# Derek-TH-Wang/OpenRoboRL

Hardware: AMD Instinct MI355X
Metric: env steps/sec at N parallel robots (higher is better)
Workload: dtype f32

## Files before the change

### openroborl_amd/csrc/orr_env_kernels.h

```cpp
#pragma once
#if defined(ORR_PHASE_TIMERS) && !defined(ORR_WAVE_TIMELINE)
#define ORR_WAVE_TIMELINE 1
#endif
#ifndef ORR_TU_MAIN
#undef ORR_PHASE_TIMERS
#endif
#include <hip/hip_runtime.h>
#include <type_traits>
#include <math.h>
#include <stdint.h>
#include <stdio.h>
#include <stdlib.h>
#include <string.h>

#include "orr_device.h"

#ifdef ORR_PHASE_TIMERS
__device__ long long g_phase_cycles[orr::kPhaseSlots];
__device__ long long g_wave_phases[2048 * 40];
#define PT_INIT() do { if (threadIdx.x == 0) { for (int i_ = 0; i_ < orr::kPhaseSlots; i_++) S.pt_acc[i_] = 0; S.pt_last = clock64(); } } while (0)
#define PT(k) do { if (threadIdx.x == 0) { const long long t_ = clock64(); S.pt_acc[k] += t_ - S.pt_last; S.pt_last = clock64(); } } while (0)
#define PT_FLUSH() do { if (threadIdx.x == 0 && blockIdx.x == gridDim.x / 2) for (int i_ = 0; i_ < orr::kPhaseSlots; i_++) atomicAdd((unsigned long long*)&g_phase_cycles[i_], (unsigned long long)S.pt_acc[i_]); \
                        if (threadIdx.x == 0 && blockIdx.x < 2048) for (int i_ = 0; i_ < orr::kPhaseSlots; i_++) g_wave_phases[blockIdx.x * 40 + i_] = S.pt_acc[i_]; } while (0)
#else
// ... 168 lines not shown
    const bool any_bad = ((__ballot(bad_act) >> (sub * kLanes)) & ((1ull << (kLanes - 1)) * 2ull - 1ull)) != 0ull;
    if (lane == 0 && any_bad) S.s[kHead - 1] = 1.0f;
  }
  if (lane < 12) {
    const float act = act_in + m_init;
    S.s[O(LAST_ACTION) + lane] = act;
    float x1 = S.s[O(XHIST) + lane], x2 = S.s[O(XHIST) + 12 + lane], y1 = S.s[O(YHIST) + lane], y2 = S.s[O(YHIST) + 12 + lane];
    if (geti(S, O(STATE_ACTION_COUNTER)) == 0) {
      const float d = map_pi(S.co[lane]);
      x1 = x2 = y1 = y2 = d;
    }
    const float y = act * P.fb[0] + (x1 * P.fb[1] + x2 * P.fb[2]) - (y1 * P.fa[1] + y2 * P.fa[2]);
    S.s[O(XHIST) + 12 + lane] = x1; S.s[O(XHIST) + lane] = act;
    S.s[O(YHIST) + 12 + lane] = y1; S.s[O(YHIST) + lane] = y;
    S.s[O(ACTION) + lane] = y;
  }
  WSYNC();
  PT(1);
  int fall = 0;
  const float inv_repeat = 1.0f / (float)c.action_repeat;
  const RingLatency rlat = ring_latency(P, S);
  const float m_gain = m_tsign * S.s[O(STRENGTH) + ml];
  const float m_target = S.s[O(ACTION) + ml], m_prev = S.s[O(FILTER_ACTION) + ml];
  const bool m_has_prev = geti(S, O(FILTER_VALID)) != 0;
  int action_counter = geti(S, O(STATE_ACTION_COUNTER));
  RingCursor ring = {geti(S, O(RING_HEAD)), geti(S, O(RING_LEN))};
  OwnCoord X;
  load_own_coord(S, lane, X);
  int limit_idle = 0;
  const int prio_phase = WPE == 2 ? (int)(((unsigned)wave_id / (unsigned)(P.simds > 0 ? P.simds : 1)) & 1u) : 0;
  const bool prio_turns = WPE == 2 && ((((unsigned)gridDim.x + (unsigned)(P.simds > 0 ? P.simds : 1) - 1u) /
                                        (unsigned)(P.simds > 0 ? P.simds : 1)) & 1u) == 0u;
  float co_own = S.co[ml], qm_c = (S.s[O(Q) + mj] - m_off) * m_dir, qdm_c = S.s[O(QD) + mj] * m_dir;
  for (int sstep = 0; sstep < c.action_repeat; sstep++) {
    constexpr int kPrioTurn = 4, kPrioHi = 1, kPrioOffset = 1, kPrioEqualFrom = 1000;
    if (WPE == 2 && prio_turns) { if (sstep < kPrioEqualFrom && ((((sstep + kPrioOffset) / kPrioTurn) ^ prio_phase) & 1)) __builtin_amdgcn_s_setprio(kPrioHi); else __builtin_amdgcn_s_setprio(0); }
    {
      const float lerp = (float)(sstep + 1) * inv_repeat;
      const float cur = map_pi(co_own);
      const float prev = m_has_prev ? m_prev : cur;
      float cmd = prev + lerp * (m_target - prev);
      cmd = fminf(fmaxf(cmd, cur - c.max_angle_change), cur + c.max_angle_change);
      S.tau[lane < 12 ? mj : lane] = m_gain * (-1.0f * (m_kp * (qm_c - cmd)) - m_kd * qdm_c);
    }
    WSYNC();
    action_counter++;
    PT(2);
    {
      RingFetch F;
      ring_prefetch(rlat, rec, ring, lane, F);
      if constexpr ((MODE & 3) == 2) {
        const size_t slot = (size_t)robot * c.action_repeat + sstep;
        if (lane < 12 && valid) RP.tau_out[slot * 12 + lane] = S.tau[mj] * m_tsign;
        WSYNC();
        for (int i = lane; i < 37; i += kLanes) S.s[O(POS) + i] = RP.traj[slot * 37 + i];
        WSYNC();
        fall = RP.fall[robot];
      } else
      fall = physics_substep<ANCHOR>(P, S, K, lane, sub, sstep == c.action_repeat - 1, X, limit_idle, ANCHOR ? &AS : nullptr, anchor_robot);
      accumulate_contacts();
      qm_c = (S.s[O(Q) + mj] - m_off) * m_dir;
      qdm_c = S.s[O(QD) + mj] * m_dir;
      ring_push_and_ctrl_obs(rec, S, lane, valid, F, ring, qm_c, &co_own);
    }
    PT(10);
  }
  if (WPE == 2) __builtin_amdgcn_s_setprio(3);
  const ResetConst RC = load_reset_const(P, S, lane);
  if (lane == 0) {
    seti(S, O(RING_HEAD), ring.head); seti(S, O(RING_LEN), ring.len);
    seti(S, O(STATE_ACTION_COUNTER), action_counter);
    seti(S, O(FILTER_VALID), 1);
    seti(S, O(STEP_COUNTER), geti(S, O(STEP_COUNTER)) + 1);
  }
  if (lane < 12) S.s[O(FILTER_ACTION) + lane] = m_target;
  WSYNC();
  sensors_push(S, lane, false);
  PT(11);
  const DevClip& clip = S.clip;
  double t = motion_time(P, S);
  double t_phase = t;
  bool switched = false;
  if constexpr (CLIPS) {
    if (t >= (double)clip_change) {
      typedef const int __attribute__((address_space(1)))* gip;
      typedef const float __attribute__((address_space(1)))* gfp;
      const int type = geti(S, O(ROBOT_TYPE));
      const int set_n = ((gip)&P.tab->clip_set_n[0])[type];
      const float sw_min = ((gfp)&P.tab->clip_switch[type][0])[0], sw_max = ((gfp)&P.tab->clip_switch[type][0])[1];
      if (set_n > 1 && sw_max < INFINITY) {
        float u4[4];
        philox_block(c.seed, (uint32_t)geti(S, O(ROBOT_INDEX)), (uint32_t)geti(S, O(EPISODE_IDX)), 8u + (uint32_t)geti(S, O(EP_STEP)), u4);
        const uint32_t m = (uint32_t)(u4[0] * 16777216.0f);
        const int k = (int)((m * (uint32_t)set_n) >> 24);
        const int id = ((gip)&P.tab->clip_set[type][0])[k];
        clip_change = clip_change_time(t, sw_min, sw_max, u4[1]);
// ... 363 lines not shown
```

### openroborl_amd/csrc/orr_physics.h

```cpp
#pragma once


__device__ __forceinline__ void chol6(const float A[36], float L[21], float invdiag[6]) {
#pragma unroll
  for (int i = 0; i < 6; i++) {
#pragma unroll
    for (int j = 0; j <= i; j++) {
      float s = A[i * 6 + j];
#pragma unroll
      for (int k = 0; k < j; k++) s -= L[i * (i + 1) / 2 + k] * L[j * (j + 1) / 2 + k];
      if (i == j) {
        const float rs = rsq(s);
        L[i * (i + 1) / 2 + j] = s * rs;
        invdiag[i] = rs;
      } else {
        L[i * (i + 1) / 2 + j] = s * invdiag[j];
      }
    }
  }
}
__device__ __forceinline__ void chol6_solve(const float L[21], const float invdiag[6], const float b[6], float x[6]) {
  float y[6];
#pragma unroll
  for (int i = 0; i < 6; i++) {
// ... 50 lines not shown
  const pk2 c3b = a3b * r3;
  d4a = pk_nfma(c3b, c3b.x, d4a);
  d5 = fmaf(-c3b.y, c3b.y, d5);
  const float r4 = rsq(d4a.x);
  const float l54 = d4a.y * r4;
  d5 = fmaf(-l54, l54, d5);
  F.idg[0] = r0; F.idg[1] = r1; F.idg[2] = r2; F.idg[3] = r3; F.idg[4] = r4; F.idg[5] = rsq(d5);
  F.l10 = l10; F.l32 = l32; F.l54 = l54;
  F.c0a = c0a; F.c0b = c0b; F.c1a = c1a; F.c1b = c1b; F.c2b = c2b; F.c3b = c3b;
}
__device__ __forceinline__ void chol6_solve_pk(const Chol6Pk& F, float b0, float b1, pk2 b23, pk2 b45, float x[6]) {
  float y[6];
  y[0] = b0 * F.idg[0];
  b1 = fmaf(-F.l10, y[0], b1); b23 = pk_nfma(F.c0a, y[0], b23); b45 = pk_nfma(F.c0b, y[0], b45);
  y[1] = b1 * F.idg[1];
  b23 = pk_nfma(F.c1a, y[1], b23); b45 = pk_nfma(F.c1b, y[1], b45);
  y[2] = b23.x * F.idg[2];
  b23.y = fmaf(-F.l32, y[2], b23.y); b45 = pk_nfma(F.c2b, y[2], b45);
  y[3] = b23.y * F.idg[3];
  b45 = pk_nfma(F.c3b, y[3], b45);
  y[4] = b45.x * F.idg[4];
  b45.y = fmaf(-F.l54, y[4], b45.y);
  y[5] = b45.y * F.idg[5];
  x[5] = y[5] * F.idg[5];
  x[4] = fmaf(-F.l54, x[5], y[4]) * F.idg[4];
  x[3] = fmaf(-F.c3b.y, x[5], fmaf(-F.c3b.x, x[4], y[3])) * F.idg[3];
  x[2] = fmaf(-F.c2b.y, x[5], fmaf(-F.c2b.x, x[4], fmaf(-F.l32, x[3], y[2]))) * F.idg[2];
  x[1] = fmaf(-F.c1b.y, x[5], fmaf(-F.c1b.x, x[4], fmaf(-F.c1a.y, x[3], fmaf(-F.c1a.x, x[2], y[1])))) * F.idg[1];
  x[0] = fmaf(-F.c0b.y, x[5], fmaf(-F.c0b.x, x[4], fmaf(-F.c0a.y, x[3], fmaf(-F.c0a.x, x[2], fmaf(-F.l10, x[1], y[0]))))) * F.idg[0];
}

#ifdef ORR_TU_STEP_W2
constexpr bool kCarrySubtreeMass = false, kOwnLegFactor = false, kPackedVelocityUpdate = false;
#define ORR_COMMON(x) (x)
#define ORR_RARE(x) (x)
#else
constexpr bool kCarrySubtreeMass = true, kOwnLegFactor = true, kPackedVelocityUpdate = true;
#define ORR_COMMON(x) __builtin_expect(!!(x), 1)
#define ORR_RARE(x) __builtin_expect(!!(x), 0)
#endif
struct LegConst {
  float r[3][3], jdir[3], joff[3];
  float com[3], m, Ic[6];
  float msub;
  float damp_l, damp_a;
  float jdir_own, joff_own;
  float int_c0, int_c1;
};
struct OwnCoord { float x0, x1; };
__device__ __forceinline__ void load_own_coord(const Shared& S, int lane, OwnCoord& X) {
  X.x0 = lane < 3 ? 0.0f : (lane < 6 ? S.s[O(POS) + lane - 3] : S.s[O(Q) + lane - 6]);
  X.x1 = lane < 2 ? S.s[O(Q) + 10 + lane] : 0.0f;
}
__device__ __forceinline__ float part_suffix_sum(float x);
__device__ static void load_leg_const(const KParams& P, const Shared& S, int lane, LegConst& K) {
  const int leg = lane & 3, part = (lane >> 2) & 3, own = 3 * leg + (part < 3 ? part : 2);
  const ColdPtr mc = model_cold(P, geti(S, O(ROBOT_TYPE)));
#pragma unroll
  for (int k = 0; k < 3; k++) {
    const int j = 3 * leg + k;
    const bool on = k <= part && part < 3;
#pragma unroll
    for (int i = 0; i < 3; i++) K.r[k][i] = on ? S.m.joint_pos[j][i] : 0.0f;
    K.jdir[k] = on ? S.m.jdir[j] : 0.0f;
    K.joff[k] = S.m.joff[j];
  }
  const bool real = part < 3, base = lane == 12;
  const int body = real ? own + 1 : 0;
#pragma unroll
  for (int i = 0; i < 3; i++) K.com[i] = real ? mc->link_com[own][i] : 0.0f;
// ... 86 lines not shown
  float t0, t1, t2;
  if constexpr (WITH_M) {
    asm("v_mov_b32 %0, 0\n\tv_mov_b32 %1, 0\n\tv_mov_b32 %2, 0\n\t"
        ORR_H_ADD("%0", "%4", "4", "0xb") ORR_H_ADD("%1", "%5", "4", "0xb") ORR_H_ADD("%2", "%6", "4", "0xb")
        "v_fmac_f32 %0, %3, %7\n\tv_fmac_f32 %1, %3, %8\n\tv_fmac_f32 %2, %3, %9\n\t"
        ORR_SUBTREE_ADD("%3", "4", "0xb")
        ORR_H_ADD("%0", "%4", "8", "0xd") ORR_H_ADD("%1", "%5", "8", "0xd") ORR_H_ADD("%2", "%6", "8", "0xd")
        ORR_SUBTREE_ADD("%3", "8", "0xd")
        : "=&v"(t0), "=&v"(t1), "=&v"(t2), "+v"(m)
        : "v"(h[0]), "v"(h[1]), "v"(h[2]), "v"(c[0]), "v"(c[1]), "v"(c[2]));
  } else {
    asm("v_mov_b32 %0, 0\n\tv_mov_b32 %1, 0\n\tv_mov_b32 %2, 0\n\t"
        ORR_H_ADD("%0", "%4", "4", "0xb") ORR_H_ADD("%1", "%5", "4", "0xb") ORR_H_ADD("%2", "%6", "4", "0xb")
        "v_fmac_f32 %0, %3, %7\n\tv_fmac_f32 %1, %3, %8\n\tv_fmac_f32 %2, %3, %9\n\t"
        ORR_H_ADD("%0", "%4", "8", "0xd") ORR_H_ADD("%1", "%5", "8", "0xd") ORR_H_ADD("%2", "%6", "8", "0xd")
        : "=&v"(t0), "=&v"(t1), "=&v"(t2)
        : "v"(m), "v"(h[0]), "v"(h[1]), "v"(h[2]), "v"(c[0]), "v"(c[1]), "v"(c[2]));
  }
  h[0] = t0; h[1] = t1; h[2] = t2;
}
#undef ORR_H_ADD
__device__ __forceinline__ void part_suffix_sum_inplace(float (&v)[6]) {
  static_assert(kRPW == 4, "a robot is one DPP row: lane = leg + 4 part, part = DPP bank");
  asm("s_nop 1\n\t"
      ORR_SUBTREE_ADD("%0", "4", "0xb") ORR_SUBTREE_ADD("%1", "4", "0xb") ORR_SUBTREE_ADD("%2", "4", "0xb")
      ORR_SUBTREE_ADD("%3", "4", "0xb") ORR_SUBTREE_ADD("%4", "4", "0xb") ORR_SUBTREE_ADD("%5", "4", "0xb")
      ORR_SUBTREE_ADD("%0", "8", "0xd") ORR_SUBTREE_ADD("%1", "8", "0xd") ORR_SUBTREE_ADD("%2", "8", "0xd")
      ORR_SUBTREE_ADD("%3", "8", "0xd") ORR_SUBTREE_ADD("%4", "8", "0xd") ORR_SUBTREE_ADD("%5", "8", "0xd")
      : "+v"(v[0]), "+v"(v[1]), "+v"(v[2]), "+v"(v[3]), "+v"(v[4]), "+v"(v[5]));
}
#undef ORR_SUBTREE_ADD

struct BaseFactor { Chol6Pk F; };
__device__ static void leg_dynamics(const KParams& P, Shared& S, const LegConst& K, int lane, BaseFactor& BF) {
  const int leg = lane & 3, part = (lane >> 2) & 3;
  float Rb[9];
#pragma unroll
  for (int i = 0; i < 9; i++) Rb[i] = S.Rb[i];
  const float wb[3] = {S.s[O(ANGVEL)], S.s[O(ANGVEL) + 1], S.s[O(ANGVEL) + 2]};
  const float vb[3] = {S.s[O(LINVEL)], S.s[O(LINVEL) + 1], S.s[O(LINVEL) + 2]};
  float Rw[9], d[3] = {0, 0, 0}, Vw[3] = {wb[0], wb[1], wb[2]}, Vv[3] = {vb[0], vb[1], vb[2]};
  float Aa[3] = {0, 0, 0}, Al[3] = {0, 0, 0};
  float s0[3], sv0[3], s1[3], sv1[3], s2[3], sv2[3], ad0, ad1, ad2;
#pragma unroll
  for (int i = 0; i < 9; i++) Rw[i] = Rb[i];
  float sn0, cs0, sn1, cs1, sn2, cs2;
  {
    const int jo = 3 * leg + (part < 3 ? part : 2);
    float sno, cso;
    joint_sincos(K.jdir_own * (S.s[O(Q) + jo] - K.joff_own), &sno, &cso);
    const float sA = __int_as_float(__builtin_amdgcn_update_dpp(0, __float_as_int(sno), 0x114, 0xF, 0xF, true));
    const float cA = __int_as_float(__builtin_amdgcn_update_dpp(0, __float_as_int(cso), 0x114, 0xF, 0xF, true));
    const float sB = __int_as_float(__builtin_amdgcn_update_dpp(0, __float_as_int(sno), 0x118, 0xF, 0xF, true));
    const float cB = __int_as_float(__builtin_amdgcn_update_dpp(0, __float_as_int(cso), 0x118, 0xF, 0xF, true));
    sn0 = __int_as_float(__builtin_amdgcn_update_dpp(__float_as_int(sno), __float_as_int(sno), 0x114, 0xF, 0x2, false));
    sn0 = __int_as_float(__builtin_amdgcn_update_dpp(__float_as_int(sn0), __float_as_int(sno), 0x118, 0xF, 0x4, false));
    cs0 = __int_as_float(__builtin_amdgcn_update_dpp(__float_as_int(cso), __float_as_int(cso), 0x114, 0xF, 0x2, false));
    cs0 = __int_as_float(__builtin_amdgcn_update_dpp(__float_as_int(cs0), __float_as_int(cso), 0x118, 0xF, 0x4, false));
    sn1 = __int_as_float(__builtin_amdgcn_update_dpp(__float_as_int(sno), __float_as_int(sno), 0x114, 0xF, 0x5, true));
    cs1 = __int_as_float(__builtin_amdgcn_update_dpp(__float_as_int(cso), __float_as_int(cso), 0x114, 0xF, 0x4, false));
    cs1 = part == 0 ? 1.0f : cs1;
    (void)sA; (void)cA; (void)sB; (void)cB;
    sn2 = part == 2 ? sno : 0.0f;
    cs2 = part == 2 ? cso : 1.0f;
  }
  float c0k[3];
  joint_down<0>(S, K, 0, 3 * leg, sn0, cs0, Rw, d, Vw, Vv, Aa, Al, s0, sv0, ad0);
  joint_down<1>(S, K, 1, 3 * leg + 1, sn1, cs1, Rw, d, Vw, Vv, Aa, Al, s1, sv1, ad1, c0k);
  joint_down<1, true>(S, K, 2, 3 * leg + 2, sn2, cs2, Rw, d, Vw, Vv, Aa, Al, s2, sv2, ad2, c0k);
  float so[3], svo[3];
#pragma unroll
  for (int i = 0; i < 3; i++) {
    so[i] = part == 0 ? s0[i] : (part == 3 ? 0.0f : s2[i]);
    svo[i] = part == 0 ? sv0[i] : (part == 3 ? 0.0f : sv2[i]);
  }
  const float ado = part == 0 ? ad0 : (part == 1 ? ad1 : ad2);
  {
    LinkCache& L = S.ph.sub.dyn.lc[part < 3 ? 3 * leg + part : 12 + leg];
#pragma unroll
    for (int i = 0; i < 9; i++) L.Rw[i] = Rw[i];
#pragma unroll
    for (int i = 0; i < 3; i++) { L.ow[i] = S.s[O(POS) + i] + d[i]; L.s[i] = so[i]; L.sv[i] = svo[i]; }
  }
  float I[6], h[3], hcom[3], m = K.m, f[6], pacc[6];
  {
    float c[3];
#pragma unroll
    for (int i = 0; i < 3; i++) hcom[i] = c[i] = fmaf(Rw[3 * i], K.com[0], fmaf(Rw[3 * i + 1], K.com[1], fmaf(Rw[3 * i + 2], K.com[2], d[i])));
    h[0] = m * c[0]; h[1] = m * c[1]; h[2] = m * c[2];
    rot_sym_full(Rw, K.Ic, I);
    float Pa[3], Pl[3];
    {
      const float ux = fmaf(Vw[1], c[2], fmaf(-Vw[2], c[1], Vv[0])), uy = fmaf(Vw[2], c[0], fmaf(-Vw[0], c[2], Vv[1]));
      const float uz = fmaf(Vw[0], c[1], fmaf(-Vw[1], c[0], Vv[2]));
      Pl[0] = m * ux; Pl[1] = m * uy; Pl[2] = m * uz;
      const float ax = fmaf(Aa[1], c[2], fmaf(-Aa[2], c[1], Al[0])), ay = fmaf(Aa[2], c[0], fmaf(-Aa[0], c[2], Al[1]));
      const float az = fmaf(Aa[0], c[1], fmaf(-Aa[1], c[0], Al[2]));
      f[3] = fmaf(m, ax, Vw[1] * Pl[2] - Vw[2] * Pl[1]);
      f[4] = fmaf(m, ay, Vw[2] * Pl[0] - Vw[0] * Pl[2]);
      f[5] = fmaf(m, az, Vw[0] * Pl[1] - Vw[1] * Pl[0]);
      symv(I, Vw, Pa);
      float tx = Vw[1] * Pa[2] - Vw[2] * Pa[1], ty = Vw[2] * Pa[0] - Vw[0] * Pa[2], tz = Vw[0] * Pa[1] - Vw[1] * Pa[0];
      tx = fmaf(I[0], Aa[0], fmaf(I[3], Aa[1], fmaf(I[4], Aa[2], tx)));
      ty = fmaf(I[3], Aa[0], fmaf(I[1], Aa[1], fmaf(I[5], Aa[2], ty)));
      tz = fmaf(I[4], Aa[0], fmaf(I[5], Aa[1], fmaf(I[2], Aa[2], tz)));
      f[0] = fmaf(c[1], f[5], fmaf(-c[2], f[4], tx));
      f[1] = fmaf(c[2], f[3], fmaf(-c[0], f[5], ty));
      f[2] = fmaf(c[0], f[4], fmaf(-c[1], f[3], tz));
    }
    const float hc = h[0] * c[0] + h[1] * c[1] + h[2] * c[2];
// ... 16 lines not shown
  part_suffix_sum_first_moment<!kCarrySubtreeMass>(m, hcom, h);
  if (kCarrySubtreeMass) m = K.msub;
  float Fo[6], bo;
  {
    spatial_inertia_mul(I, h, m, so, svo, &Fo[0], &Fo[3]);
    auto dot6 = [](const float a[3], const float b[3], const float x[3], const float y[3]) __attribute__((always_inline)) {
      return fmaf(a[0], x[0], fmaf(a[1], x[1], fmaf(a[2], x[2], fmaf(b[0], y[0], fmaf(b[1], y[1], b[2] * y[2])))));
    };
    bo = S.tau[3 * leg + (part < 3 ? part : 2)] - dot6(so, svo, &f[0], &f[3]);
    const float hc0 = dot6(s0, sv0, &Fo[0], &Fo[3]), hc1 = dot6(s1, sv1, &Fo[0], &Fo[3]), hc2 = dot6(s2, sv2, &Fo[0], &Fo[3]);
    {
      LegExchange& X = S.ph.sub.dyn.legx[leg];
#pragma unroll
      for (int i = 0; i < 6; i++) X.F[part][i] = Fo[i];
      X.b[part] = bo;
      X.Hc[part][0] = hc0; X.Hc[part][1] = hc1; X.Hc[part][2] = hc2;
    }
  }
  WSYNC();
  float b[3];
  pk2 F2[3][3];
  float H00, H01, H02, H11, H12, H22;
  {
    const LegExchange& X = S.ph.sub.dyn.legx[leg];
#pragma unroll
    for (int k = 0; k < 3; k++) {
      static_assert(sizeof(X.F[0]) == 24 && alignof(LegExchange) >= 8, "pairs");
      const pk2* XF = reinterpret_cast<const pk2*>(&X.F[k][0]);
#pragma unroll
      for (int q = 0; q < 3; q++) F2[k][q] = XF[q];
      b[k] = X.b[k];
    }
    H00 = X.Hc[0][0]; H01 = X.Hc[1][0]; H11 = X.Hc[1][1]; H02 = X.Hc[2][0]; H12 = X.Hc[2][1]; H22 = X.Hc[2][2];
  }
  float Hi[6];
  {
    const float c00 = H11 * H22 - H12 * H12, c01 = H02 * H12 - H01 * H22, c02 = H01 * H12 - H02 * H11;
    const float c11 = H00 * H22 - H02 * H02, c12 = H01 * H02 - H00 * H12, c22 = H00 * H11 - H01 * H01;
    const float idet = __builtin_amdgcn_rcpf(H00 * c00 + H01 * c01 + H02 * c02);
    Hi[0] = c00 * idet; Hi[1] = c11 * idet; Hi[2] = c22 * idet; Hi[3] = c01 * idet; Hi[4] = c02 * idet; Hi[5] = c12 * idet;
  }
  const float hq0 = part == 0 ? Hi[0] : (part == 1 ? Hi[3] : (part == 2 ? Hi[4] : 0.0f));
  const float hq1 = part == 0 ? Hi[3] : (part == 1 ? Hi[1] : (part == 2 ? Hi[5] : 0.0f));
  const float hq2 = part == 0 ? Hi[4] : (part == 1 ? Hi[5] : (part == 2 ? Hi[2] : 0.0f));
  float Tq[6];
  pk2 Tq2[3];
#pragma unroll
  for (int q = 0; q < 3; q++) { Tq2[q] = F2[0][q] * hq0 + F2[1][q] * hq1 + F2[2][q] * hq2; Tq[2 * q] = Tq2[q].x; Tq[2 * q + 1] = Tq2[q].y; }
  {
    LegSolve& Q = S.leg[leg];
    float* const tdst = part < 3 ? &Q.T[part][0] : &S.tdump[0];
#pragma unroll
    for (int q = 0; q < 3; q++) reinterpret_cast<pk2*>(tdst)[q] = Tq2[q];
#pragma unroll
    for (int i = 0; i < 6; i++) Q.Hi[i] = Hi[i];
  }
  float a0[6];
  {
    const pk2 Fo23 = {Fo[2], Fo[3]}, Fo45 = {Fo[4], Fo[5]};
    float d0 = fmaf(-Tq[0], Fo[0], Iacc[0]), a10 = fmaf(-Tq[0], Fo[1], Iacc[3]);
    pk2 a0a = pk_nfma(Fo23, Tq[0], pk2{Iacc[4], Hacc[0]}), a0b = pk_nfma(Fo45, Tq[0], pk2{Hacc[1], Hacc[2]});
    float d1 = fmaf(-Tq[1], Fo[1], Iacc[1]);
    pk2 a1a = pk_nfma(Fo23, Tq[1], pk2{Iacc[5], Hacc[3]}), a1b = pk_nfma(Fo45, Tq[1], pk2{Hacc[4], Hacc[5]});
    pk2 d2a = pk_nfma(Fo23, Tq[2], pk2{Iacc[2], Hacc[6]}), a2b = pk_nfma(Fo45, Tq[2], pk2{Hacc[7], Hacc[8]});
    float d3 = fmaf(-Tq[3], Fo[3], Macc[0]);
    pk2 a3b = pk_nfma(Fo45, Tq[3], pk2{Macc[3], Macc[4]});
// ... 142 lines not shown
    else { G.c20 = cr[0]; G.c21 = cr[1]; G.c22 = cr[2]; }
    jl[k] = dir[0] * cr[0] + dir[1] * cr[1] + dir[2] * cr[2];
    rel += jl[k] * S.ustar[6 + 3 * leg + k];
  }
  G.rr0 = rr[0]; G.rr1 = rr[1]; G.rr2 = rr[2];
  const bool active = enable && (knee ? fr > 0.0f : have);
#pragma unroll
  for (int i = 0; i < 6; i++) R.Jb[i] = knee ? 0.0f : Jb[i];
  R.jl[0] = knee ? 0.0f : jl[0]; R.jl[1] = knee ? 0.0f : jl[1]; R.jl[2] = knee ? 1.0f : jl[2];
  const float kpen = normal ? (dist > 0.0f ? inv_dt : (shank ? erp_dt : erp_m)) : 0.0f;
  float rhs = knee ? -uknee : -rel - dist * kpen;
  if constexpr (ANCHOR) rhs -= (d == 1 ? drift_x : (d == 2 ? drift_y : 0.0f)) * (cfg.friction_erp * inv_dt);
  R.rhs = active ? rhs : 0.0f;
  R.cfm = (normal && !shank) ? cfm_m : 0.0f;
  R.nrm_slot = fric ? 16 + leg : -1;
  R.warm = knee ? -1 : 3 * leg + d;
  R.active = active;
  R.jdi = 0.0f; R.lam = 0.0f; R.w = 0.0f; R.lam_n = 0.0f;
  const float hi = knee ? fr * dt : 1e30f, lo = knee ? -fr * dt : 0.0f;
  R.mu_e = (active && fric) ? mu_s * cfg.plane_friction : 0.0f;
  R.hi_c = (active && !fric) ? hi : 0.0f;
  R.lo_c = (active && !fric) ? lo : 0.0f;
}

typedef float v2f __attribute__((ext_vector_type(2)));
__device__ __forceinline__ void row_response(Shared& S, const orr_config& cfg, Row& R, int slot, const BaseFactor& BF) {
  const int leg = R.leg;
  const LegSolve& QL = S.leg[leg];
  float a0[6], mq[12];
  v2f fb2[3], a02[3];
  float prev = S.s[O(LAMBDA) + (R.warm >= 0 ? R.warm : 0)];
  float jl0 = R.jl[0], jl1 = R.jl[1], jl2 = R.jl[2];
  asm("" : "+v"(jl0), "+v"(jl1), "+v"(jl2));
  {
    const v2f* TL = reinterpret_cast<const v2f*>(&QL.T[0][0]);
#pragma unroll
    for (int p = 0; p < 3; p++) {
      float jb0 = R.Jb[2 * p], jb1 = R.Jb[2 * p + 1];
      asm("" : "+v"(jb0), "+v"(jb1));
      const v2f jb = {jb0, jb1};
      fb2[p] = jb - (TL[p] * jl0 + TL[3 + p] * jl1 + TL[6 + p] * jl2);
    }
    chol6_solve_pk(BF.F, fb2[0].x, fb2[0].y, fb2[1], fb2[2], a0);
#pragma unroll
    for (int p = 0; p < 3; p++) a02[p] = v2f{a0[2 * p], a0[2 * p + 1]};
  }
  asm volatile("" : "+v"(prev));
  const float h0 = QL.Hi[0] * jl0 + QL.Hi[3] * jl1 + QL.Hi[4] * jl2;
  const float h1 = QL.Hi[3] * jl0 + QL.Hi[1] * jl1 + QL.Hi[5] * jl2;
  const float h2 = QL.Hi[4] * jl0 + QL.Hi[5] * jl1 + QL.Hi[2] * jl2;
  const v2f dg = fb2[0] * a02[0] + fb2[1] * a02[1] + fb2[2] * a02[2];
  float dgs = dg.x + dg.y;
  asm volatile("" : "+v"(dgs));
  const float own0 = leg == 0 ? 1.0f : 0.0f, own1 = leg == 1 ? 1.0f : 0.0f, own2 = leg == 2 ? 1.0f : 0.0f, own3 = leg == 3 ? 1.0f : 0.0f;
#pragma unroll
  for (int L4 = 0; L4 < 4; L4++) {
    const v2f* TK = reinterpret_cast<const v2f*>(&S.leg[L4].T[0][0]);
    const float own = L4 == 0 ? own0 : (L4 == 1 ? own1 : (L4 == 2 ? own2 : own3));
#pragma unroll
    for (int k = 0; k < 3; k++) {
      const v2f t2 = TK[3 * k] * a02[0] + TK[3 * k + 1] * a02[1] + TK[3 * k + 2] * a02[2];
      const float hk = k == 0 ? h0 : (k == 1 ? h1 : h2);
      mq[3 * L4 + k] = kOwnLegFactor ? fmaf(own, hk, -(t2.x + t2.y)) : ((L4 == leg ? hk : 0.0f) - (t2.x + t2.y));
    }
  }
  const float diag = fmaf(jl0, h0, fmaf(jl1, h1, fmaf(jl2, h2, dgs)));
#pragma unroll
  for (int i = 0; i < 6; i++) S.ph.sub.W[slot][i] = a0[i];
#pragma unroll
  for (int i = 0; i < 12; i++) S.ph.sub.W[slot][6 + i] = mq[i];
#pragma unroll
  for (int i = 0; i < 6; i++) R.wa[i] = a0[i];
#pragma unroll
  for (int i = 0; i < 12; i++) R.wq[i] = mq[i];
  R.jdi = R.active ? __builtin_amdgcn_rcpf(diag + R.cfm) : 0.0f;
  R.rhs *= R.jdi;
  {
    asm volatile("" : "+v"(prev));
    R.lam = (R.active && R.warm >= 0) ? cfg.warmstart_factor * prev : 0.0f;
    R.w = R.cfm * R.lam;
  }
}

template <int I, int N, class F>
__device__ __forceinline__ void static_for(F&& f) {
  if constexpr (I < N) {
    f(std::integral_constant<int, I>{});
    static_for<I + 1, N>(f);
  }
}
template <class F>
__device__ __forceinline__ void for_active_limit_rows(unsigned int mask, F&& f) {
  static_for<0, 4>([&](auto gc) __attribute__((always_inline)) {
    constexpr int g = decltype(gc)::value;
// ... 234 lines not shown
    }
    asm("" : "+v"(AcA[r]), "+v"(AcB[r]));
  };
  static_for<0, 4>([&](auto rc) __attribute__((always_inline)) {
    constexpr int r = decltype(rc)::value;
    finish(rc, A.wq[3 * r + 2], HAS_B ? B.wq[3 * r + 2] : 0.0f);
  });
  if (HAS_B) {
    for_active_limit_rows(mask, [&](auto rc) __attribute__((always_inline)) {
      constexpr int r = decltype(rc)::value;
      const float sg = bcast_lane<r>(B.jl[(r - 4) % 3], sub);
      finish(rc, sg * A.wq[r - 4], sg * B.wq[r - 4]);
    });
  }
  const unsigned int cm = (mask >> 16) & 0xFu;
  static_for<0, 4>([&](auto gc) __attribute__((always_inline)) {
    constexpr int g = decltype(gc)::value;
    if (ORR_COMMON((cm >> g) & 1u)) {
      float ax, ay, az, bx = 0.0f, by = 0.0f, bz = 0.0f;
      dpp_contact_triplet<4 + g>(G.rr0, G.rr1, G.rr2, G.c00, G.c01, G.c02, G.c10, G.c11, G.c12, G.c20, G.c21, G.c22, A.wa[0], A.wa[1], A.wa[2],
                                 A.wa[3], A.wa[4], A.wa[5], A.wq[3 * g], A.wq[3 * g + 1], A.wq[3 * g + 2], ax, ay, az);
      if (HAS_B)
        dpp_contact_triplet<4 + g>(G.rr0, G.rr1, G.rr2, G.c00, G.c01, G.c02, G.c10, G.c11, G.c12, G.c20, G.c21, G.c22, B.wa[0], B.wa[1], B.wa[2],
                                   B.wa[3], B.wa[4], B.wa[5], B.wq[3 * g], B.wq[3 * g + 1], B.wq[3 * g + 2], bx, by, bz);
      finish(std::integral_constant<int, 16 + g>{}, az, bz);
      finish(std::integral_constant<int, 20 + 2 * g>{}, ax, bx);
      finish(std::integral_constant<int, 21 + 2 * g>{}, ay, by);
    }
  });
}

template <bool ANCHOR = false>
__device__ static int physics_substep(const KParams& P, Shared& S, const LegConst& K, int lane, int sub, bool want_fall, OwnCoord& X,
                                      int& limit_idle, AnchorState* AS = nullptr, bool anchor_robot = false) {
  const orr_config& cfg = P.cfg;
  const float dt = cfg.sim_dt, inv_dt = 1.0f / cfg.sim_dt, erp_dt = cfg.contact_erp / cfg.sim_dt;
  int fp_body = 0, fp_n = 0;
  float fp_x = 0.0f, fp_y = 0.0f, fp_z = 0.0f, fp_r = 0.0f;
  if (ORR_RARE(want_fall)) {
    const ColdPtr mc = model_cold(P, geti(S, O(ROBOT_TYPE)));
    static_assert(ORR_MAX_FALL_PROXIES <= kLanes, "one fall proxy per lane");
    fp_body = mc->fall_body[lane]; fp_x = mc->fall_pos[lane][0]; fp_y = mc->fall_pos[lane][1]; fp_z = mc->fall_pos[lane][2]; fp_r = mc->fall_radius[lane];
    fp_n = mc->num_fall;
  }
  BaseFactor BF;
  leg_dynamics(P, S, K, lane, BF);
  WSYNC();
  PT(3);
  asm volatile("" : "+v"(fp_n));
  int fall = 0;
  if (ORR_RARE(want_fall)) {
    bool hit = false;
    if (lane < fp_n) {
      const int b = fp_body;
      const float* Rw = b == 0 ? S.Rb : S.ph.sub.dyn.lc[b - 1].Rw;
      const float oz = b == 0 ? S.s[O(POS) + 2] : S.ph.sub.dyn.lc[b - 1].ow[2];
      const float wz = Rw[6] * fp_x + Rw[7] * fp_y + Rw[8] * fp_z;
      hit = (oz + wz - fp_r) < cfg.contact_margin;
    }
    fall = ((__ballot(hit) >> (sub * kLanes)) & ((1ull << (kLanes - 1)) * 2ull - 1ull)) != 0ull;
  }
  PT(4);

  Row A, B;
  const bool rowlane = lane < 16;
  ContactGeom G;
  row_setup_bank_a<ANCHOR>(S, cfg, rowlane ? (lane < 4 ? lane : lane + 12) : 0, rowlane, dt, inv_dt, erp_dt, A, G, AS, anchor_robot);
  unsigned long long balB = 0ull;
  if (ORR_COMMON(limit_idle > 0)) {
    limit_idle--;
    B.active = false;
  } else {
    float margin = 1e30f;
    row_setup_limit(S, cfg, (rowlane && lane >= 4) ? lane : 4, rowlane && lane >= 4, inv_dt, erp_dt, B, &margin);
    balB = __ballot(B.active);
    const float steps_f = (rowlane && lane >= 4) ? margin * __builtin_amdgcn_rcpf(cfg.max_coord_velocity * dt) - 1.0f : 1e30f;
    int idle = 0;
    if (__ballot(steps_f < 1.0f) == 0ull) idle = 1;
    if (__ballot(steps_f < 2.0f) == 0ull) idle = 2;
// ... 68 lines not shown
      };
      static_for<0, 4>(add_row);
      if (anyB) {
        for_active_limit_rows(mask, add_row);
      }
      static_for<16, 28>(add_row);
    }
    const float vmax = cfg.max_coord_velocity;
    v0 = __builtin_amdgcn_fmed3f(S.ustar[k0] + du0, -vmax, vmax);
    v1 = __builtin_amdgcn_fmed3f(S.ustar[k1] + du1, -vmax, vmax);
  }
  {
    const float w0 = bcast_lane<0>(v0, sub), w1 = bcast_lane<1>(v0, sub), w2 = bcast_lane<2>(v0, sub);
    const float ww = w0 * w0 + w1 * w1 + w2 * w2, h2 = 0.25f * dt * dt * ww;
    const float sc = 0.5f * dt * fmaf(h2, fmaf(h2, fmaf(h2, -1.0f / 5040.0f, 1.0f / 120.0f), -1.0f / 6.0f), 1.0f);
    const float ch = fmaf(h2, fmaf(h2, fmaf(h2, fmaf(h2, 1.0f / 40320.0f, -1.0f / 720.0f), 1.0f / 24.0f), -0.5f), 1.0f);
    const float dq[4] = {w0 * sc, w1 * sc, w2 * sc, ch};
    float qn[4];
    qmul(dq, &S.s[O(QUAT)], qn);
    const float nn = rsq(qn[0] * qn[0] + qn[1] * qn[1] + qn[2] * qn[2] + qn[3] * qn[3]);
    X.x0 = fmaf(dt * v0, K.int_c0, X.x0);
    X.x1 = fmaf(dt * v1, K.int_c1, X.x1);
    float* const dump = &S.ustar[22];
    float* const pv0 = &S.s[lane < 3 ? O(ANGVEL) + lane : (lane < 6 ? O(LINVEL) + lane - 3 : O(QD) + lane - 6)];
    float* const px0 = lane < 3 ? dump : &S.s[lane < 6 ? O(POS) + lane - 3 : O(Q) + lane - 6];
    float* const pv1 = lane < 2 ? &S.s[O(QD) + 10 + lane] : dump;
    float* const px1 = lane < 2 ? &S.s[O(Q) + 10 + lane] : dump;
    float* const pq = lane < 4 ? &S.s[O(QUAT) + lane] : dump;
    WSYNC();
    *pv0 = lane < 6 ? v0 : v0 * K.int_c0;
    *px0 = X.x0;
    *pv1 = v1 * K.int_c1;
    *px1 = X.x1;
    *pq = pick4(lane, qn[0], qn[1], qn[2], qn[3]) * nn;
  }
  WSYNC();
  PT(9);
  return fall;
}
```

### openroborl_amd/csrc/orr_robot_io.h

```cpp
#pragma once

typedef float f4 __attribute__((ext_vector_type(4)));
__device__ static void load_robot(const KParams& P, const float* rec, Shared& S, int lane) {
  {
    static_assert(kHead % 4 == 0 && ORR_STATE_STRIDE % 4 == 0, "16-byte pieces");
    typedef const f4 __attribute__((address_space(1))) * g4ptr;
    const g4ptr src = (g4ptr)reinterpret_cast<const f4*>(rec);
    f4* dst = reinterpret_cast<f4*>(S.s);
    constexpr int kQ = kHead / 4, kIt = (kQ + kLanes - 1) / kLanes;
    f4 tmp[kIt];
#pragma unroll
    for (int k = 0; k < kIt; k++) { const int q = lane + k * kLanes; tmp[k] = src[q < kQ ? q : kQ - 1]; }
#pragma unroll
    for (int k = 0; k < kIt; k++) { const int q = lane + k * kLanes; if (q < kQ) dst[q] = tmp[k]; }
  }
  WSYNC();
  const DevModel& gm = P.tab->model[geti(S, O(ROBOT_TYPE))];
  {
    static_assert(sizeof(DevClip) % 4 == 0 && sizeof(DevClip) / 4 <= kLanes, "one word of the clip header per lane");
    const unsigned int* cg = reinterpret_cast<const unsigned int*>(&P.tab->clip[geti(S, O(CLIP_ID))]);
    unsigned int* cl = reinterpret_cast<unsigned int*>(&S.clip);
    if (lane < (int)(sizeof(DevClip) / 4)) cl[lane] = cg[lane];
  }
  {
// ... 11 lines not shown
  WSYNC();
}

__device__ static void store_robot(float* rec, const Shared& S, int lane, bool valid) {
  if (valid) {
    typedef f4 __attribute__((address_space(1))) * g4ptr;
    const g4ptr dst = (g4ptr)reinterpret_cast<f4*>(rec);
    const f4* src = reinterpret_cast<const f4*>(S.s);
    constexpr int kQ = O(RING) / 4;
#pragma unroll
    for (int k = 0; k < (kQ + kLanes - 1) / kLanes; k++) { const int q = lane + k * kLanes; if (q < kQ) dst[q] = src[q]; }
    if (lane < O(RING) - 4 * kQ) rec[4 * kQ + lane] = S.s[4 * kQ + lane];
  }
}

__device__ static void ctrl_obs(const KParams& P, const float* rec, Shared& S, int lane) {
  const float lat = S.s[O(LATENCY)], dt = P.cfg.sim_dt;
  const int len = geti(S, O(RING_LEN)), head = geti(S, O(RING_HEAD));
  int k0 = 0, k1 = 0;
  float al = 0.0f;
  if (!(lat <= 0.0f || len == 1)) {
    int n = (int)(lat / dt);
    if (n + 1 >= len) { k0 = k1 = len - 1; }
    else { k0 = n; k1 = n + 1; al = (lat - n * dt) / dt; }
  }
  const int i0 = (head - k0 + 2 * ORR_RING_DEPTH) % ORR_RING_DEPTH, i1 = (head - k1 + 2 * ORR_RING_DEPTH) % ORR_RING_DEPTH;
  for (int i = lane; i < 19; i += kLanes) {
    float e0 = rec[O(RING) + i0 * ORR_RING_ENTRY + i], e1 = rec[O(RING) + i1 * ORR_RING_ENTRY + i];
    S.co[i] = (k0 == k1) ? e0 : (1.0f - al) * e0 + al * e1;
  }
  WSYNC();
}

__device__ __forceinline__ void base_rotation(Shared& S, int lane, float rel[4], float Rb[9]) {
  float qi[4];
  qinv(S.m.init_quat, qi);
  qmul(&S.s[O(QUAT)], qi, rel);
  q_to_mat(rel, Rb);
#pragma unroll
  for (int i = 0; i < 9; i++) S.Rb[i] = Rb[i];
}

struct ResetConst {
  int j;
  float off, dir;
  float init;
  float p0;
};
__device__ __forceinline__ ResetConst load_reset_const(const KParams& P, const Shared& S, int lane) {
  const ColdPtr mc = model_cold(P, geti(S, O(ROBOT_TYPE)));
  const int ml = lane < 12 ? lane : 0;
  return ResetConst{mc->joint_of_motor[ml], mc->motor_offset[ml], mc->motor_dir[ml], mc->init_motor_angles[ml], mc->init_pos[lane < 3 ? lane : 0]};
}

__device__ static void receive_obs(const KParams& P, float* rec, Shared& S, int lane, bool valid, const ResetConst& RC, float* entry = nullptr) {
  const int head = (geti(S, O(RING_HEAD)) + 1) % ORR_RING_DEPTH, len = geti(S, O(RING_LEN));
  float rel[4], Rb[9], rate[3];
  base_rotation(S, lane, rel, Rb);
  mtv3(Rb, &S.s[O(ANGVEL)], rate);
  for (int i = lane; i < ORR_RING_ENTRY; i += kLanes) {
    float val = 0.0f;
    if (i < 12) {
      static_assert(kLanes >= 12, "the first pass of the loop covers the twelve motors");
      val = (S.s[O(Q) + RC.j] - RC.off) * RC.dir;
    } else if (i < 16) {
      val = i == 12 ? rel[0] : (i == 13 ? rel[1] : (i == 14 ? rel[2] : rel[3]));
    } else if (i < 19) {
      val = i == 16 ? rate[0] : (i == 17 ? rate[1] : rate[2]);
    }
    if (valid) rec[O(RING) + head * ORR_RING_ENTRY + i] = val;
// ... 16 lines not shown
  int n;
  float al;
  bool none;
};
__device__ __forceinline__ RingLatency ring_latency(const KParams& P, const Shared& S) {
  const float lat = S.s[O(LATENCY)], dt = P.cfg.sim_dt;
  RingLatency L;
  L.none = lat <= 0.0f;
  L.n = (int)(lat / dt);
  L.al = (lat - L.n * dt) / dt;
  return L;
}
struct RingCursor { int head, len; };
__device__ __forceinline__ int ring_wrap_up(int i) { return i >= ORR_RING_DEPTH ? i - ORR_RING_DEPTH : i; }
__device__ __forceinline__ int ring_wrap_down(int i) { return i < 0 ? i + ORR_RING_DEPTH : i; }
__device__ __forceinline__ void ring_prefetch(const RingLatency& L, const float* rec, const RingCursor& C, int lane, RingFetch& F) {
  const int head = ring_wrap_up(C.head + 1);
  const int len = C.len + 1 > ORR_RING_DEPTH ? ORR_RING_DEPTH : C.len + 1;
  int k0 = 0, k1 = 0;
  F.al = 0.0f;
  if (!(L.none || len == 1)) {
    if (L.n + 1 >= len) { k0 = k1 = len - 1; }
    else { k0 = L.n; k1 = L.n + 1; F.al = L.al; }
  }
  F.same = k0 == k1; F.new0 = k0 == 0; F.new1 = k1 == 0;
  const int i0 = ring_wrap_down(head - k0), i1 = ring_wrap_down(head - k1);
  const float* p0 = rec + O(RING) + i0 * ORR_RING_ENTRY;
  const float* p1 = rec + O(RING) + i1 * ORR_RING_ENTRY;
  const int hi = lane < 3 ? 16 + lane : lane;
  F.e0[0] = p0[lane]; F.e0[1] = p0[hi];
  F.e1[0] = p1[lane]; F.e1[1] = p1[hi];
}
__device__ __forceinline__ void ring_push_and_ctrl_obs(float* rec, Shared& S, int lane, bool valid, const RingFetch& F, RingCursor& C,
                                                       float mang, float* co_own = nullptr) {
  static_assert(ORR_RING_ENTRY == 20, "lane mapping below assumes 20-word entries");
  C.head = ring_wrap_up(C.head + 1);
  C.len = C.len + 1 > ORR_RING_DEPTH ? ORR_RING_DEPTH : C.len + 1;
  float rel[4], Rb[9], rate[3];
  base_rotation(S, lane, rel, Rb);
  mtv3(Rb, &S.s[O(ANGVEL)], rate);
  const float va = lane < 12 ? mang : pick4(lane, rel[0], rel[1], rel[2], rel[3]);
  const float vb = pick4(lane, rate[0], rate[1], rate[2], 0.0f);
  const float a0 = F.new0 ? va : F.e0[0], a1 = F.new1 ? va : F.e1[0];
  const float b0 = F.new0 ? vb : F.e0[1], b1 = F.new1 ? vb : F.e1[1];
  const float co_a = F.same ? a0 : (1.0f - F.al) * a0 + F.al * a1;
  S.co[lane] = co_a;
  if (co_own) *co_own = co_a;
  S.co[lane < 3 ? 16 + lane : 19] = F.same ? b0 : (1.0f - F.al) * b0 + F.al * b1;
  WSYNC();
  float* dst = rec + O(RING) + C.head * ORR_RING_ENTRY;
  if (valid) {
    dst[lane] = va;
    dst[lane < 4 ? 16 + lane : lane] = lane < 4 ? vb : va;
  }
}
```

Measured before the change: 21.74 million.

## Carry base state in registers and hoist LDS reads ahead of waits

Keeps the integrated base quaternion and angular velocity in registers and hands them to the observation step, which avoids re-reading them from LDS. The inverse of the initial quaternion is computed once per step instead of once per substep. Rb and the own joint angle are prefetched before the wave sync, the link-cache writes are moved after the Hessian work, and the first leg's T rows are loaded ahead in the contact response so LDS latency overlaps compute. The cost is higher register pressure, and the scheduling barriers could work against the compiler's own ordering.

```diff
diff --git a/openroborl_amd/csrc/orr_env_kernels.h b/openroborl_amd/csrc/orr_env_kernels.h
--- a/openroborl_amd/csrc/orr_env_kernels.h
+++ b/openroborl_amd/csrc/orr_env_kernels.h
@@ -224,7 +224,16 @@
   const bool prio_turns = WPE == 2 && ((((unsigned)gridDim.x + (unsigned)(P.simds > 0 ? P.simds : 1) - 1u) /
                                         (unsigned)(P.simds > 0 ? P.simds : 1)) & 1u) == 0u;
   float co_own = S.co[ml], qm_c = (S.s[O(Q) + mj] - m_off) * m_dir, qdm_c = S.s[O(QD) + mj] * m_dir;
+  BaseHandoff BH;
+  BH.has_qi = kCarryInitQuatInverse;
+  if (BH.has_qi) qinv(S.m.init_quat, BH.qi);
   for (int sstep = 0; sstep < c.action_repeat; sstep++) {
+    LegHead LH;
+    if (kLegHeadAhead) {
+#pragma unroll
+      for (int i = 0; i < 9; i++) LH.Rb[i] = S.Rb[i];
+      LH.q = S.s[O(Q) + 3 * (lane & 3) + (((lane >> 2) & 3) < 3 ? ((lane >> 2) & 3) : 2)];
+    }
     constexpr int kPrioTurn = 4, kPrioHi = 1, kPrioOffset = 1, kPrioEqualFrom = 1000;
     if (WPE == 2 && prio_turns) { if (sstep < kPrioEqualFrom && ((((sstep + kPrioOffset) / kPrioTurn) ^ prio_phase) & 1)) __builtin_amdgcn_s_setprio(kPrioHi); else __builtin_amdgcn_s_setprio(0); }
     {
@@ -236,11 +245,15 @@
       S.tau[lane < 12 ? mj : lane] = m_gain * (-1.0f * (m_kp * (qm_c - cmd)) - m_kd * qdm_c);
     }
     WSYNC();
+    if (kLegHeadAhead)
+      asm volatile("" : "+v"(LH.Rb[0]), "+v"(LH.Rb[1]), "+v"(LH.Rb[2]), "+v"(LH.Rb[3]), "+v"(LH.Rb[4]), "+v"(LH.Rb[5]), "+v"(LH.Rb[6]), "+v"(LH.Rb[7]),
+                        "+v"(LH.Rb[8]), "+v"(LH.q));
     action_counter++;
     PT(2);
     {
       RingFetch F;
       ring_prefetch(rlat, rec, ring, lane, F);
+      constexpr bool kHandoff = kBaseHandoff && (MODE & 3) != 2;
       if constexpr ((MODE & 3) == 2) {
         const size_t slot = (size_t)robot * c.action_repeat + sstep;
         if (lane < 12 && valid) RP.tau_out[slot * 12 + lane] = S.tau[mj] * m_tsign;
@@ -249,11 +262,11 @@
         WSYNC();
         fall = RP.fall[robot];
       } else
-      fall = physics_substep<ANCHOR>(P, S, K, lane, sub, sstep == c.action_repeat - 1, X, limit_idle, ANCHOR ? &AS : nullptr, anchor_robot);
+      fall = physics_substep<ANCHOR>(P, S, K, lane, sub, sstep == c.action_repeat - 1, X, limit_idle, ANCHOR ? &AS : nullptr, anchor_robot, kHandoff ? &BH : nullptr, kLegHeadAhead ? &LH : nullptr);
       accumulate_contacts();
       qm_c = (S.s[O(Q) + mj] - m_off) * m_dir;
       qdm_c = S.s[O(QD) + mj] * m_dir;
-      ring_push_and_ctrl_obs(rec, S, lane, valid, F, ring, qm_c, &co_own);
+      ring_push_and_ctrl_obs(rec, S, lane, valid, F, ring, qm_c, &co_own, kHandoff ? &BH : nullptr);
     }
     PT(10);
   }
diff --git a/openroborl_amd/csrc/orr_physics.h b/openroborl_amd/csrc/orr_physics.h
--- a/openroborl_amd/csrc/orr_physics.h
+++ b/openroborl_amd/csrc/orr_physics.h
@@ -106,10 +106,12 @@
 
 #ifdef ORR_TU_STEP_W2
 constexpr bool kCarrySubtreeMass = false, kOwnLegFactor = false, kPackedVelocityUpdate = false;
+constexpr bool kBaseHandoff = false, kCarryInitQuatInverse = false, kExchangeShadow = false, kLegHeadAhead = false, kRowResponseAhead = false;
 #define ORR_COMMON(x) (x)
 #define ORR_RARE(x) (x)
 #else
 constexpr bool kCarrySubtreeMass = true, kOwnLegFactor = true, kPackedVelocityUpdate = true;
+constexpr bool kBaseHandoff = true, kCarryInitQuatInverse = true, kExchangeShadow = true, kLegHeadAhead = true, kRowResponseAhead = true;
 #define ORR_COMMON(x) __builtin_expect(!!(x), 1)
 #define ORR_RARE(x) __builtin_expect(!!(x), 0)
 #endif
@@ -262,11 +264,11 @@
 #undef ORR_SUBTREE_ADD
 
 struct BaseFactor { Chol6Pk F; };
-__device__ static void leg_dynamics(const KParams& P, Shared& S, const LegConst& K, int lane, BaseFactor& BF) {
+__device__ static void leg_dynamics(const KParams& P, Shared& S, const LegConst& K, int lane, BaseFactor& BF, const LegHead* LH = nullptr) {
   const int leg = lane & 3, part = (lane >> 2) & 3;
   float Rb[9];
 #pragma unroll
-  for (int i = 0; i < 9; i++) Rb[i] = S.Rb[i];
+  for (int i = 0; i < 9; i++) Rb[i] = LH ? LH->Rb[i] : S.Rb[i];
   const float wb[3] = {S.s[O(ANGVEL)], S.s[O(ANGVEL) + 1], S.s[O(ANGVEL) + 2]};
   const float vb[3] = {S.s[O(LINVEL)], S.s[O(LINVEL) + 1], S.s[O(LINVEL) + 2]};
   float Rw[9], d[3] = {0, 0, 0}, Vw[3] = {wb[0], wb[1], wb[2]}, Vv[3] = {vb[0], vb[1], vb[2]};
@@ -278,7 +280,7 @@
   {
     const int jo = 3 * leg + (part < 3 ? part : 2);
     float sno, cso;
-    joint_sincos(K.jdir_own * (S.s[O(Q) + jo] - K.joff_own), &sno, &cso);
+    joint_sincos(K.jdir_own * ((LH ? LH->q : S.s[O(Q) + jo]) - K.joff_own), &sno, &cso);
     const float sA = __int_as_float(__builtin_amdgcn_update_dpp(0, __float_as_int(sno), 0x114, 0xF, 0xF, true));
     const float cA = __int_as_float(__builtin_amdgcn_update_dpp(0, __float_as_int(cso), 0x114, 0xF, 0xF, true));
     const float sB = __int_as_float(__builtin_amdgcn_update_dpp(0, __float_as_int(sno), 0x118, 0xF, 0xF, true));
@@ -305,7 +307,12 @@
     svo[i] = part == 0 ? sv0[i] : (part == 3 ? 0.0f : sv2[i]);
   }
   const float ado = part == 0 ? ad0 : (part == 1 ? ad1 : ad2);
-  {
+  float lc_ow[3];
+  if constexpr (kExchangeShadow) {
+#pragma unroll
+    for (int i = 0; i < 3; i++) lc_ow[i] = S.s[O(POS) + i] + d[i];
+  }
+  if constexpr (!kExchangeShadow) {
     LinkCache& L = S.ph.sub.dyn.lc[part < 3 ? 3 * leg + part : 12 + leg];
 #pragma unroll
     for (int i = 0; i < 9; i++) L.Rw[i] = Rw[i];
@@ -388,6 +395,14 @@
       b[k] = X.b[k];
     }
     H00 = X.Hc[0][0]; H01 = X.Hc[1][0]; H11 = X.Hc[1][1]; H02 = X.Hc[2][0]; H12 = X.Hc[2][1]; H22 = X.Hc[2][2];
+  }
+  if constexpr (kExchangeShadow) {
+    LinkCache& L = S.ph.sub.dyn.lc[part < 3 ? 3 * leg + part : 12 + leg];
+#pragma unroll
+    for (int i = 0; i < 9; i++) L.Rw[i] = Rw[i];
+#pragma unroll
+    for (int i = 0; i < 3; i++) { L.ow[i] = lc_ow[i]; L.s[i] = so[i]; L.sv[i] = svo[i]; }
+    asm volatile("" : "+v"(H00), "+v"(H01), "+v"(H02), "+v"(H11), "+v"(H12), "+v"(H22) : : "memory");
   }
   float Hi[6];
   {
@@ -596,6 +611,12 @@
   float prev = S.s[O(LAMBDA) + (R.warm >= 0 ? R.warm : 0)];
   float jl0 = R.jl[0], jl1 = R.jl[1], jl2 = R.jl[2];
   asm("" : "+v"(jl0), "+v"(jl1), "+v"(jl2));
+  v2f tk0[9];
+  if constexpr (kRowResponseAhead) {
+    const v2f* TK = reinterpret_cast<const v2f*>(&S.leg[0].T[0][0]);
+#pragma unroll
+    for (int i = 0; i < 9; i++) tk0[i] = TK[i];
+  }
   {
     const v2f* TL = reinterpret_cast<const v2f*>(&QL.T[0][0]);
 #pragma unroll
@@ -610,6 +631,7 @@
     for (int p = 0; p < 3; p++) a02[p] = v2f{a0[2 * p], a0[2 * p + 1]};
   }
   asm volatile("" : "+v"(prev));
+  if constexpr (kRowResponseAhead) asm volatile("" : "+v"(tk0[0]), "+v"(tk0[1]), "+v"(tk0[2]), "+v"(tk0[3]), "+v"(tk0[4]), "+v"(tk0[5]), "+v"(tk0[6]), "+v"(tk0[7]), "+v"(tk0[8]));
   const float h0 = QL.Hi[0] * jl0 + QL.Hi[3] * jl1 + QL.Hi[4] * jl2;
   const float h1 = QL.Hi[3] * jl0 + QL.Hi[1] * jl1 + QL.Hi[5] * jl2;
   const float h2 = QL.Hi[4] * jl0 + QL.Hi[5] * jl1 + QL.Hi[2] * jl2;
@@ -623,7 +645,8 @@
     const float own = L4 == 0 ? own0 : (L4 == 1 ? own1 : (L4 == 2 ? own2 : own3));
 #pragma unroll
     for (int k = 0; k < 3; k++) {
-      const v2f t2 = TK[3 * k] * a02[0] + TK[3 * k + 1] * a02[1] + TK[3 * k + 2] * a02[2];
+      const bool pre = kRowResponseAhead && L4 == 0;
+      const v2f t2 = (pre ? tk0[3 * k] : TK[3 * k]) * a02[0] + (pre ? tk0[3 * k + 1] : TK[3 * k + 1]) * a02[1] + (pre ? tk0[3 * k + 2] : TK[3 * k + 2]) * a02[2];
       const float hk = k == 0 ? h0 : (k == 1 ? h1 : h2);
       mq[3 * L4 + k] = kOwnLegFactor ? fmaf(own, hk, -(t2.x + t2.y)) : ((L4 == leg ? hk : 0.0f) - (t2.x + t2.y));
     }
@@ -924,7 +947,7 @@
 
 template <bool ANCHOR = false>
 __device__ static int physics_substep(const KParams& P, Shared& S, const LegConst& K, int lane, int sub, bool want_fall, OwnCoord& X,
-                                      int& limit_idle, AnchorState* AS = nullptr, bool anchor_robot = false) {
+                                      int& limit_idle, AnchorState* AS = nullptr, bool anchor_robot = false, BaseHandoff* BH = nullptr, const LegHead* LH = nullptr) {
   const orr_config& cfg = P.cfg;
   const float dt = cfg.sim_dt, inv_dt = 1.0f / cfg.sim_dt, erp_dt = cfg.contact_erp / cfg.sim_dt;
   int fp_body = 0, fp_n = 0;
@@ -936,7 +959,7 @@
     fp_n = mc->num_fall;
   }
   BaseFactor BF;
-  leg_dynamics(P, S, K, lane, BF);
+  leg_dynamics(P, S, K, lane, BF, LH);
   WSYNC();
   PT(3);
   asm volatile("" : "+v"(fp_n));
@@ -1071,7 +1094,13 @@
     *px0 = X.x0;
     *pv1 = v1 * K.int_c1;
     *px1 = X.x1;
-    *pq = pick4(lane, qn[0], qn[1], qn[2], qn[3]) * nn;
+    if (kBaseHandoff && BH) {
+      BH->q[0] = qn[0] * nn; BH->q[1] = qn[1] * nn; BH->q[2] = qn[2] * nn; BH->q[3] = qn[3] * nn;
+      BH->w[0] = w0; BH->w[1] = w1; BH->w[2] = w2;
+      *pq = pick4(lane, BH->q[0], BH->q[1], BH->q[2], BH->q[3]);
+    } else {
+      *pq = pick4(lane, qn[0], qn[1], qn[2], qn[3]) * nn;
+    }
   }
   WSYNC();
   PT(9);
diff --git a/openroborl_amd/csrc/orr_robot_io.h b/openroborl_amd/csrc/orr_robot_io.h
--- a/openroborl_amd/csrc/orr_robot_io.h
+++ b/openroborl_amd/csrc/orr_robot_io.h
@@ -67,10 +67,14 @@
   WSYNC();
 }
 
-__device__ __forceinline__ void base_rotation(Shared& S, int lane, float rel[4], float Rb[9]) {
+struct BaseHandoff { float q[4], w[3]; float qi[4]; bool has_qi; };
+struct LegHead { float Rb[9], q; };
+__device__ __forceinline__ void base_rotation(Shared& S, int lane, float rel[4], float Rb[9], const BaseHandoff* BH = nullptr) {
   float qi[4];
-  qinv(S.m.init_quat, qi);
-  qmul(&S.s[O(QUAT)], qi, rel);
+  if (BH && BH->has_qi) { qi[0] = BH->qi[0]; qi[1] = BH->qi[1]; qi[2] = BH->qi[2]; qi[3] = BH->qi[3]; }
+  else qinv(S.m.init_quat, qi);
+  if (BH) qmul(BH->q, qi, rel);
+  else qmul(&S.s[O(QUAT)], qi, rel);
   q_to_mat(rel, Rb);
 #pragma unroll
   for (int i = 0; i < 9; i++) S.Rb[i] = Rb[i];
@@ -153,13 +157,13 @@
   F.e1[0] = p1[lane]; F.e1[1] = p1[hi];
 }
 __device__ __forceinline__ void ring_push_and_ctrl_obs(float* rec, Shared& S, int lane, bool valid, const RingFetch& F, RingCursor& C,
-                                                       float mang, float* co_own = nullptr) {
+                                                       float mang, float* co_own = nullptr, const BaseHandoff* BH = nullptr) {
   static_assert(ORR_RING_ENTRY == 20, "lane mapping below assumes 20-word entries");
   C.head = ring_wrap_up(C.head + 1);
   C.len = C.len + 1 > ORR_RING_DEPTH ? ORR_RING_DEPTH : C.len + 1;
   float rel[4], Rb[9], rate[3];
-  base_rotation(S, lane, rel, Rb);
-  mtv3(Rb, &S.s[O(ANGVEL)], rate);
+  base_rotation(S, lane, rel, Rb, BH);
+  mtv3(Rb, BH ? BH->w : &S.s[O(ANGVEL)], rate);
   const float va = lane < 12 ? mang : pick4(lane, rel[0], rel[1], rel[2], rel[3]);
   const float vb = pick4(lane, rate[0], rate[1], rate[2], 0.0f);
   const float a0 = F.new0 ? va : F.e0[0], a1 = F.new1 ? va : F.e1[0];
```

After: 21.95 million, median of 6. No clear change (+1.0%).
